# alvinliu0/HumanGaussian

Measured on AMD Instinct MI355X. Metric: rasterize fwd+bwd Gaussians/sec @1024^2, 100k pts, higher is better.
Workload: dtype f32

## Files before the change

### humangaussian_amd/csrc/api.hip

```cpp
#include "hgs_common.h"
#include <stdio.h>
#include <stdlib.h>
#include <algorithm>
#include <atomic>
#include <mutex>

#ifdef HGS_TIMELINE
__device__ unsigned long long hgs_tl[HGS_TL_KERNELS][HGS_TL_SLOTS][4];
#endif
#include "preprocess.hip"
#include "binning.hip"
#include "render_fwd.hip"
#include "knn.hip"
#include "mesh.hip"
#include "fields.hip"
#include "bookkeeping.hip"
#include "optim.hip"

extern "C" __global__ void hgs_k_render_bwd(View, Layout, const hgs_status*, const SortRec*, const float*,
                                            const float*, const float*, const float*, const float*,
                                            const float*, const float*, float*, uint32_t);
extern "C" __global__ void hgs_k_pair_reduce_em(View, Layout, const hgs_status*, const SortRec*, const float*, float*, uint32_t, uint32_t);
extern "C" __global__ void hgs_k_pair_reduce_ch(View, Layout, const hgs_status*, const SortRec*, const float*, float*, uint32_t, uint32_t);

// ... 92 lines not shown
  const BinCarve b = carve_bin(cap);
  char* gp = static_cast<char*>(geom);
  char* bp = static_cast<char*>(bin);
  Layout L;
  L.geom = reinterpret_cast<GeomRec*>(gp + g.geom);
  L.tile_n = reinterpret_cast<uint32_t*>(gp + g.tile_n);
  L.tile_start = reinterpret_cast<uint32_t*>(gp + g.tile_start);
  L.tile_order = reinterpret_cast<uint32_t*>(gp + g.tile_order);
  L.tile_rec = reinterpret_cast<uint4*>(gp + g.tile_rec);
  L.cell_info = reinterpret_cast<CellInfo*>(gp + g.cell_info);
  L.items_part = reinterpret_cast<uint4*>(gp + g.items_part);
  L.fwd_cells = reinterpret_cast<uint32_t*>(gp + g.fwd_cells);
  L.hist = reinterpret_cast<uint32_t*>(gp + g.hist);
  L.tile_gbase = reinterpret_cast<uint32_t*>(gp + g.tile_gbase);
  L.tile_count = reinterpret_cast<uint32_t*>(gp + g.tile_count);
  L.chunk_sums = reinterpret_cast<uint32_t*>(gp + g.chunk_sums);
  L.chunk_base = reinterpret_cast<uint32_t*>(gp + g.chunk_base);
  L.ctr = reinterpret_cast<Counters*>(gp + g.ctr);
  L.keys = bp ? reinterpret_cast<unsigned long long*>(bp + b.keys) : nullptr;
  L.recs = bp ? reinterpret_cast<SortRec*>(bp + b.recs) : nullptr;
  L.cell_list = bp ? reinterpret_cast<uint2*>(bp + b.cell_list) : nullptr;
  L.entpair = bp ? reinterpret_cast<uint2*>(bp + b.entpair) : nullptr;
  L.cstate = bp ? reinterpret_cast<float*>(bp + b.cstate) : nullptr;
  L.items_full = bp ? reinterpret_cast<uint4*>(bp + b.items_full) : nullptr;
  L.full_cap = (uint32_t)((size_t)(cap > 0 ? cap : 0) * HGS_PAIRS_PER_ENTRY / HGS_SEGLEN + 1);
  L.n_contrib = static_cast<uint32_t*>(img);
  return L;
}

View make_view(const hgs_settings* s, int B, int P, int M, int64_t cap, int max_tile_hint = 0, int act = 0) {
// ... 47 lines not shown
#define HGS_STAGE(k)                                                              \
  do {                                                                            \
    if (stage_events && stage_events[k]) {                                        \
      hipError_t e__ = hipEventRecord(static_cast<hipEvent_t>(stage_events[k]), stream); \
      if (e__ != hipSuccess) return hip_rc(e__);                                  \
    }                                                                             \
  } while (0)

struct SideStream {
  std::mutex mu;
  hipStream_t s = nullptr;
  hipEvent_t fork = nullptr, join = nullptr;
  bool tried = false, ok = false;
};

struct DeviceState {
  std::atomic<int> cus;
  SideStream side;
  std::atomic<int> lds_raised[HGS_PRE_BWD_ROWS];
};
DeviceState g_devices[64];
DeviceState* device_state(hipStream_t stream) {
  int dev = 0;
  if (hipStreamGetDevice(stream, &dev) != hipSuccess || dev < 0 || dev >= 64) { (void)hipGetLastError(); return nullptr; }
  return &g_devices[dev];
}
struct DeviceCurrent {
  int dev, cur = 0;
  bool ok, switched;
  explicit DeviceCurrent(const DeviceState* ds)
      : dev((int)(ds - g_devices)), ok(hipGetDevice(&cur) == hipSuccess), switched(ok && cur != dev) {
    if (switched) ok = hipSetDevice(dev) == hipSuccess;
  }
  ~DeviceCurrent() { if (switched) (void)hipSetDevice(cur); }
};

int cu_count(DeviceState* ds) {
  if (!ds) return 256;
  int cus = ds->cus.load(std::memory_order_relaxed);
  if (cus > 0) return cus;
  if (hipDeviceGetAttribute(&cus, hipDeviceAttributeMultiprocessorCount, (int)(ds - g_devices)) != hipSuccess || cus < 1) cus = 256;
  ds->cus.store(cus, std::memory_order_relaxed);
  return cus;
}

SideStream* side_stream(DeviceState* ds) {
  if (!ds) return nullptr;
  SideStream& t = ds->side;
  std::lock_guard<std::mutex> lk(t.mu);
  if (!t.tried) {
    t.tried = true;
    DeviceCurrent on(ds);
    t.ok = on.ok && hipStreamCreateWithFlags(&t.s, hipStreamNonBlocking) == hipSuccess &&
           hipEventCreateWithFlags(&t.fork, hipEventDisableTiming) == hipSuccess &&
           hipEventCreateWithFlags(&t.join, hipEventDisableTiming) == hipSuccess;
    if (!t.ok) (void)hipGetLastError();
  }
  return t.ok ? &t : nullptr;
// ... 215 lines not shown
    if ((shs != nullptr) == (colors_precomp != nullptr)) return HGS_ESHAPE;
    const bool has_sr = scales != nullptr && rotations != nullptr;
    if ((scales != nullptr) != (rotations != nullptr)) return HGS_ESHAPE;
    if (has_sr == (cov3D_precomp != nullptr)) return HGS_ESHAPE;
    if (shs && M < (s->sh_degree + 1) * (s->sh_degree + 1)) return HGS_ESHAPE;
    if (entry_capacity > 0 && !bin) return HGS_EINVAL;
    if ((int64_t)B * P >= (1ll << 31) || P >= (1 << 28)) return HGS_EINVAL;
  }
  if (entry_capacity > HGS_MAX_ENTRY_CAPACITY) return HGS_EINVAL;
  hipStream_t stream = static_cast<hipStream_t>(stream_);
  DeviceState* const ds = device_state(stream);
  const int ncu = cu_count(ds);
  const bool aa = (activation_flags & HGS_ANTIALIAS) != 0;
  const View v = make_view(s, B, P, M, entry_capacity, max_tile_entries_hint > 0 ? max_tile_entries_hint : 0,
                           activation_flags & 7);
  const Layout L = make_layout(geom, bin, img, B, P, v.H, v.W, entry_capacity);
  hgs_status* status_dev =
      reinterpret_cast<hgs_status*>(static_cast<char*>(geom) + carve_geom(B, P, v.H, v.W).status);

  HGS_STAGE(0);
  hipError_t e = hipSuccess;
  if (v.nblk == 0) {
    e = hipMemsetAsync(L.ctr, 0, sizeof(Counters), stream);
    if (e != hipSuccess) return hip_rc(e);
  }
  const size_t lds_bytes = (size_t)v.T * 4;
  if (!v.lds_bins) {
    e = hipMemsetAsync(L.tile_count, 0, (size_t)v.TT * 4, stream);
    if (e != hipSuccess) return hip_rc(e);
  }
  if (v.nblk > 0) {
    if (v.lds_bins)
      hipLaunchKernelGGL(aa ? hgs_k_preprocess_fwd_aa : hgs_k_preprocess_fwd, dim3(v.B * v.nwg), dim3(HGS_BLOCK), lds_bytes,
                         stream, v, L, means3D, shs, colors_precomp, opacities, scales, rotations,
                         cov3D_precomp, radii, means2D_leaf);
    else
      hipLaunchKernelGGL(aa ? hgs_k_preprocess_fwd_ga_aa : hgs_k_preprocess_fwd_ga, dim3(v.B * v.nblk), dim3(HGS_BLOCK), 0,
                         stream, v, L, means3D, shs, colors_precomp, opacities, scales, rotations,
                         cov3D_precomp, radii, means2D_leaf);
    HGS_LAUNCH_CHECK();
  }
  HGS_STAGE(1);
  const unsigned bpv = (unsigned)((v.T + HGS_TILES_PER_WG - 1) / HGS_TILES_PER_WG);
  hipLaunchKernelGGL(hgs_k_tiles, dim3(bpv * (unsigned)v.B), dim3(64 * HGS_ROW_GROUPS), 0, stream, v, L);
  HGS_LAUNCH_CHECK();
  HGS_STAGE(2);
  const unsigned order_wgs = (unsigned)((v.TT + HGS_BLOCK - 1) / HGS_BLOCK);
  hgs_status* status_mapped = status_host_mapped ? status_host : nullptr;
  const unsigned nbin = entry_capacity > 0 ? (unsigned)(v.B * (v.lds_bins ? v.nwg : v.nblk)) : 0u;
  if (v.lds_bins && nbin)
    hipLaunchKernelGGL(hgs_k_fill, dim3(nbin + order_wgs), dim3(HGS_BLOCK), lds_bytes, stream, v, L, status_dev,
                       status_mapped, (int)nbin);
  else
    hipLaunchKernelGGL(hgs_k_fill_ga, dim3(nbin + order_wgs), dim3(HGS_BLOCK), 0, stream, v, L, status_dev,
                       status_mapped, (int)nbin);
  HGS_LAUNCH_CHECK();
  if (status_host && !status_host_mapped) {
    e = hipMemcpyAsync(status_host, status_dev, sizeof(hgs_status), hipMemcpyDeviceToHost, stream);
    if (e != hipSuccess) return hip_rc(e);
  }
// ... 44 lines not shown
    }
  } else {
    HGS_STAGE(3);
  }
  HGS_STAGE(4);
  {
    const int64_t cells = std::min<int64_t>((int64_t)16 * v.TT, (int64_t)HGS_PAIRS_PER_ENTRY * entry_capacity);
    const int64_t fwd_blocks = (int64_t)hgs_knob("HGS_FWD_BLOCKS_PER_CU", 4) * ncu;
    const unsigned cell_blocks = (unsigned)std::max<int64_t>(4, std::min<int64_t>(fwd_blocks, (cells + 3) / 4) & ~int64_t(3));
    const unsigned bg_blocks = (unsigned)v.TT;
    hipLaunchKernelGGL(store_bwd_state ? hgs_k_render_fwd_store : hgs_k_render_fwd_nostore, dim3(cell_blocks + bg_blocks),
                       dim3(HGS_FWD_THREADS), 0, stream, v, L, cell_blocks, status_dev, status_mapped, L.recs, L.cstate,
                       out_color, out_depth, out_alpha);
  }
  HGS_LAUNCH_CHECK();
  HGS_STAGE(5);
  return HGS_OK;
}

int hgs_forward_batch(const hgs_settings* s, int32_t B, int32_t P, int32_t M, const float* means3D,
                      const float* shs, const float* colors_precomp, const float* opacities,
                      const float* scales, const float* rotations, const float* cov3D_precomp,
                      float* out_color, float* out_depth, float* out_alpha, int32_t* radii,
                      void* geom, void* bin, int64_t entry_capacity, void* img,
                      int32_t store_bwd_state, int32_t max_tile_entries_hint, hgs_status* status_host,
                      int32_t status_host_mapped, void* status_event, void* const* stage_events,
                      void* stream_) {
  return hgs_forward_batch_act(s, B, P, M, means3D, shs, colors_precomp, opacities, scales, rotations, cov3D_precomp,
                               out_color, out_depth, out_alpha, radii, geom, bin, entry_capacity, img, store_bwd_state,
                               max_tile_entries_hint, status_host, status_host_mapped, status_event, stage_events, 0,
// ... 546 lines not shown
```

### humangaussian_amd/csrc/binning.hip

```cpp
#include "hgs_common.h"

extern "C" __global__ void __launch_bounds__(64 * HGS_ROW_GROUPS)
hgs_k_tiles(View v, Layout L) {
  __shared__ uint32_t gt[HGS_ROW_GROUPS][HGS_TILES_PER_WG];
  __shared__ uint32_t start_s[HGS_TILES_PER_WG];
  __shared__ uint32_t cls_s[HGS_NCLS];
  const int tid = threadIdx.x, tl = tid & 63;
  const int rg = __builtin_amdgcn_readfirstlane(tid >> 6);
  const int bpv = (v.T + HGS_TILES_PER_WG - 1) / HGS_TILES_PER_WG;
  const int b = (int)blockIdx.x / bpv;
  const int t = ((int)blockIdx.x % bpv) * HGS_TILES_PER_WG + tl;
  const bool valid = t < v.T;
  const size_t g = (size_t)b * v.T + t;
  if (tid < HGS_NCLS) cls_s[tid] = 0;
  uint32_t run = 0;
  if (v.lds_bins) {
    const int rpg = (v.nwg + HGS_ROW_GROUPS - 1) / HGS_ROW_GROUPS;
    const int r0 = rg * rpg, r1 = min(v.nwg, r0 + rpg);
    if (valid) {
      uint32_t* col = L.hist + (size_t)b * v.nwg * v.T + t;
      constexpr int BR = 16;
      for (int r = r0; r < r1; r += BR) {
        uint32_t c[BR];
#pragma unroll
        for (int k = 0; k < BR; ++k) c[k] = (r + k < r1) ? col[(size_t)(r + k) * v.T] : 0u;
#pragma unroll
        for (int k = 0; k < BR; ++k) {
          if (r + k < r1 && c[k]) col[(size_t)(r + k) * v.T] = run;
          run += c[k];
        }
      }
    }
  } else if (rg == 0 && valid) {
    run = L.tile_count[g];
    L.tile_count[g] = 0;
  }
  gt[rg][tl] = run;
  __syncthreads();
  uint32_t gbase = 0;
#pragma unroll
  for (int k = 0; k < HGS_ROW_GROUPS; ++k) gbase += (k < rg) ? gt[k][tl] : 0u;
  if (rg == 0) {
    uint32_t n = 0;
#pragma unroll
    for (int k = 0; k < HGS_ROW_GROUPS; ++k) n += gt[k][tl];
    if (!valid) n = 0;
    const uint32_t i0 = hgs_wave_incl_scan(n);
    unsigned long long b_eb = 0;
    if (tl == 63 && i0) b_eb = atomicAdd(&L.ctr->alloc_eb, (unsigned long long)i0);
    const uint32_t s0 = (uint32_t)__builtin_amdgcn_readlane((int)(uint32_t)b_eb, 63);
    const uint32_t start = s0 + i0 - n;
    start_s[tl] = start;
    if (valid) {
      L.tile_n[g] = n;
      L.tile_start[g] = start;
    }
    const unsigned long long eb = __ballot(valid && n == 0);
    if (tl == 0 && eb) atomicAdd(&cls_s[0], (uint32_t)__popcll(eb));
    if (valid && n) atomicAdd(&cls_s[32 - __clz(n)], 1u);
    const uint32_t mx = hgs_wave_max_u32(n);
    if (tl == 0 && mx) atomicMax(&L.ctr->max_n, mx);
  }
  __syncthreads();
  if (v.lds_bins && valid) L.tile_gbase[(size_t)rg * v.TT + g] = start_s[tl] + gbase;
  if (tid < HGS_NCLS && cls_s[tid]) atomicAdd(&L.ctr->cls_hist[tid].v, cls_s[tid]);

}

__device__ __forceinline__ uint32_t overflow_from_counters(const View& v, const Layout& L) {
  const uint32_t R = (uint32_t)L.ctr->alloc_eb;
  uint32_t o = (R > v.entry_capacity) ? 1u : 0u;
  if (v.max_tile_hint > 0 && L.ctr->max_n > (uint32_t)v.max_tile_hint) o |= 2u;
  return o;
}

__device__ __forceinline__ void place_tiles(const View& v, const Layout& L, int blk, int nblks,
                                            hgs_status* __restrict__ status,
                                            hgs_status* __restrict__ status_host) {
  __shared__ uint32_t cls_base[HGS_NCLS];
  __shared__ uint32_t cls_cnt[HGS_NCLS];
  const int tid = threadIdx.x, lane = tid & 63;
  if (tid < HGS_NCLS) cls_cnt[tid] = L.ctr->cls_hist[tid].v;
  __syncthreads();
  if (tid == 0) {
    uint32_t acc = 0;
    for (int c = HGS_NCLS - 1; c >= 0; --c) { cls_base[c] = acc; acc += cls_cnt[c]; }
  }
  if (blk == 0 && tid == 64) {
    const unsigned long long a_eb = L.ctr->alloc_eb;
    hgs_status st;
    st.num_rendered = (uint32_t)a_eb;
    st.active_tiles = (uint32_t)v.TT - cls_cnt[0];
    st.num_pairs = 0;
    st.bwd_groups = 0;
    st.overflow = overflow_from_counters(v, L);
    st.reserved[0] = v.entry_capacity;
    st.reserved[1] = L.ctr->max_n;
    st.reserved[2] = 1;
    *status = st;
    if (status_host) {
      volatile uint32_t* hs = reinterpret_cast<volatile uint32_t*>(status_host);
      const uint32_t* sw = reinterpret_cast<const uint32_t*>(&st);
      for (int k = 0; k < 7; ++k) hs[k] = sw[k];
      __threadfence_system();
      hs[7] = 1u;
      __threadfence_system();
    }
  }
  if (tid >= 128 && tid < 192) {
    const int nchunk = v.B * v.nblk;
    const int per_wg = (nchunk + nblks - 1) / nblks;
    const int c_begin = blk * per_wg, c_end = min(nchunk, c_begin + per_wg);
    for (int c0 = c_begin; c0 < c_end; c0 += 64) {
      const int c = c0 + lane;
      const uint32_t sum = (c < c_end) ? L.chunk_sums[c] : 0u;
      const uint32_t inc = hgs_wave_incl_scan(sum);
      uint32_t base = 0;
      if (lane == 63 && inc) base = atomicAdd(&L.ctr->entry_alloc, inc);
      base = (uint32_t)__builtin_amdgcn_readlane((int)base, 63);
      if (c < c_end) L.chunk_base[c] = base + inc - sum;
    }
  }
  __syncthreads();
  const int g = blk * HGS_BLOCK + tid;
  const bool valid = g < v.TT;
  const uint32_t n = valid ? L.tile_n[g] : 0u;
  const int c = (valid && n) ? 32 - __clz(n) : 0;
  int leader_of = 0;
  uint32_t rank = 0, cnt = 0;
  unsigned long long todo = __ballot(valid);
  while (todo) {
    const int leader = (int)__builtin_ctzll(todo);
    const int cl = __builtin_amdgcn_readlane(c, leader);
    const unsigned long long same = __ballot(valid && c == cl);
    if (valid && c == cl) {
      leader_of = leader;
      rank = __builtin_amdgcn_mbcnt_hi((uint32_t)(same >> 32), __builtin_amdgcn_mbcnt_lo((uint32_t)same, 0u));
      cnt = (uint32_t)__popcll(same);
    }
    todo &= ~same;
  }
  uint32_t base = 0;
  if (valid && lane == leader_of) base = atomicAdd(&L.ctr->cls_cur[c].v, cnt);
  base = (uint32_t)__shfl((int)base, leader_of, 64);
  const uint32_t pos = cls_base[c] + base + rank;
  if (!valid) return;
  L.tile_order[pos] = (uint32_t)g;
  L.tile_rec[pos] = make_uint4((uint32_t)g, n, L.tile_start[g], 0u);
}

extern "C" __global__ void __launch_bounds__(HGS_BLOCK)
hgs_k_fill(View v, Layout L, hgs_status* __restrict__ status, hgs_status* __restrict__ status_host, int nbin) {
  extern __shared__ __attribute__((aligned(16))) uint32_t lds_cur[];
  if ((int)blockIdx.x >= nbin) {
    place_tiles(v, L, (int)blockIdx.x - nbin, (int)gridDim.x - nbin, status, status_host);
    return;
  }
  if (overflow_from_counters(v, L)) return;
  const int b = (int)blockIdx.x / v.nwg, lw = (int)blockIdx.x % v.nwg;
  const uint32_t* __restrict__ base_row = L.hist + (size_t)blockIdx.x * v.T;
  const int rpg = (v.nwg + HGS_ROW_GROUPS - 1) / HGS_ROW_GROUPS;
  const uint32_t* __restrict__ grp_row = L.tile_gbase + (size_t)(lw / rpg) * v.TT + (size_t)b * v.T;
  for (int t = threadIdx.x; t < v.T; t += HGS_BLOCK) lds_cur[t] = grp_row[t] + base_row[t];
  __syncthreads();
  const GeomRec* __restrict__ geom = L.geom + (size_t)b * v.P;
  for (int c = 0; c < v.cpw; ++c) {
    const int chunk = lw * v.cpw + c;
    if (chunk >= v.nblk) break;
    const int i = chunk * HGS_BLOCK + threadIdx.x;
    if (i >= v.P) continue;
    const uint4 q2 = reinterpret_cast<const uint4*>(&geom[i])[2];
    const uint32_t depth_bits = q2.y, lo = q2.z, hi = q2.w;
    const int minx = lo & 0xffffu, miny = lo >> 16, maxx = hi & 0xffffu, maxy = hi >> 16;
    const unsigned long long key_hi = (unsigned long long)depth_bits << 32;
    for (int ty = miny; ty < maxy; ++ty)
      for (int tx = minx; tx < maxx; ++tx) {
        const uint32_t slot = atomicAdd(&lds_cur[ty * v.grid_x + tx], 1u);
        L.keys[slot] = key_hi | (uint32_t)i;
      }
  }
}

extern "C" __global__ void __launch_bounds__(HGS_BLOCK)
hgs_k_fill_ga(View v, Layout L, hgs_status* __restrict__ status, hgs_status* __restrict__ status_host, int nbin) {
  if ((int)blockIdx.x >= nbin) {
    place_tiles(v, L, (int)blockIdx.x - nbin, (int)gridDim.x - nbin, status, status_host);
// ... 406 lines not shown
#define HGS_RANK_BUCKET_MAX 192
#define HGS_RANK_NB_MAX 2048
#define HGS_SORT_NT 256
#define HGS_SORT_WAVES_PER_EU 3
#define HGS_RANK_GU 2

namespace {

#ifdef HGS_TIMELINE
__shared__ unsigned long long hgs_s_tq[8];
#define HGS_TQ(i) { if (threadIdx.x == 0) hgs_s_tq[(i)] = wall_clock64(); }
#else
#define HGS_TQ(i) {}
#endif

__device__ __forceinline__ void lds_barrier() { asm volatile("s_waitcnt lgkmcnt(0)\n\ts_barrier" ::: "memory"); }

struct __attribute__((aligned(16))) RankLds {
  uint32_t hist[HGS_RANK_NB_MAX + 1];
  uint32_t wtot[16];
  uint32_t tot16[8];
  uint32_t dmin, dmax, maxcnt, pad;
};
static_assert(sizeof(uint32_t) * (HGS_RANK_NB_MAX + 1) >= sizeof(uint16_t) * 4096, "the masks of the longest list fit into the histogram");

template <int NT>
__device__ __forceinline__ void bucket_scan(RankLds& R, uint32_t NB) {
  int tid = (int)threadIdx.x;
  asm volatile("" : "+v"(tid));
  const int lane = tid & 63, wv = tid >> 6;
  const uint32_t PER = NB / (uint32_t)NT;
// ... 546 lines not shown
```

### humangaussian_amd/csrc/hgs_common.h

```cpp
#pragma once
#include <hip/hip_runtime.h>
#include <stdint.h>

#include "../../include/hgs_rast.h"
#include "cellmask.h"
#include "entryrec.h"

#define HGS_TILE 16
#define HGS_TILE_PIX 256
#define HGS_BLOCK 256
#define HGS_ROW_GROUPS 16
#define HGS_TILES_PER_WG 64
#define HGS_RB 16
#define HGS_ROW_F4 (HGS_RB * HGS_REC_F4 + 1)
#define HGS_BWD_BLOCK_WAVES 12
#define HGS_SEGLEN 128
#define HGS_NEAR_Z 0.2f
#define HGS_ALPHA_MIN (1.0f / 255.0f)
#define HGS_ALPHA_MAX 0.99f
#define HGS_T_EPS 0.0001f
#define HGS_CSTATE_FLOATS (6 * 16)
#define HGS_ROW_FLOATS 12
#define HGS_GROW_F4 (HGS_ROW_FLOATS / 4)
#define HGS_PROW_FLOATS 10
// ... 44 lines not shown

__host__ __device__ __forceinline__ uint32_t hgs_cell_class(uint32_t len) {
  const uint32_t nb = (len + HGS_RB - 1) / HGS_RB;
  return nb >= 33u ? 0u : nb >= 25u ? 1u : nb >= 17u ? 2u : nb >= 13u ? 3u : nb >= 9u ? 4u : nb >= 7u ? 5u : nb >= 5u ? 6u : 11u - nb;
}

struct Layout {
  GeomRec* geom;
  uint32_t* tile_n;
  uint32_t* tile_start;
  uint32_t* tile_order;
  uint4* tile_rec;
  uint32_t* hist;
  uint32_t* tile_gbase;
  uint32_t* tile_count;
  uint32_t* chunk_sums;
  uint32_t* chunk_base;
  CellInfo* cell_info;
  uint32_t* fwd_cells;
  uint4* items_part;
  Counters* ctr;
  unsigned long long* keys;
  SortRec* recs;
  uint2* cell_list;
  uint2* entpair;
  float* cstate;
  uint32_t full_cap;
  uint4* items_full;
  uint32_t* n_contrib;
};
// ... 53 lines not shown
  x += __builtin_amdgcn_update_dpp(0, x, HGS_DPP_ROW_SHR(4), 0xf, 0xf, false);
  x += __builtin_amdgcn_update_dpp(0, x, HGS_DPP_ROW_SHR(8), 0xf, 0xf, false);
  x += __builtin_amdgcn_update_dpp(0, x, HGS_DPP_ROW_BCAST15, 0xa, 0xf, false);
  x += __builtin_amdgcn_update_dpp(0, x, HGS_DPP_ROW_BCAST31, 0xc, 0xf, false);
  return (uint32_t)x;
}

__device__ __forceinline__ uint32_t hgs_wave_max_u32(uint32_t v) {
  int x = (int)v;
  x = (int)max((uint32_t)x, (uint32_t)__builtin_amdgcn_update_dpp(0, x, HGS_DPP_ROW_SHR(1), 0xf, 0xf, false));
  x = (int)max((uint32_t)x, (uint32_t)__builtin_amdgcn_update_dpp(0, x, HGS_DPP_ROW_SHR(2), 0xf, 0xf, false));
  x = (int)max((uint32_t)x, (uint32_t)__builtin_amdgcn_update_dpp(0, x, HGS_DPP_ROW_SHR(4), 0xf, 0xf, false));
  x = (int)max((uint32_t)x, (uint32_t)__builtin_amdgcn_update_dpp(0, x, HGS_DPP_ROW_SHR(8), 0xf, 0xf, false));
  x = (int)max((uint32_t)x, (uint32_t)__builtin_amdgcn_update_dpp(0, x, HGS_DPP_ROW_BCAST15, 0xa, 0xf, false));
  x = (int)max((uint32_t)x, (uint32_t)__builtin_amdgcn_update_dpp(0, x, HGS_DPP_ROW_BCAST31, 0xc, 0xf, false));
  return (uint32_t)__builtin_amdgcn_readlane(x, 63);
}

template <int NT>
__device__ __forceinline__ uint32_t hgs_block_excl_scan(uint32_t v, uint32_t* wtot,
                                                        uint32_t& total) {
  const int lane = threadIdx.x & 63, w = threadIdx.x >> 6;
  const uint32_t incl = hgs_wave_incl_scan(v);
  __syncthreads();
  if (lane == 63) wtot[w] = incl;
  __syncthreads();
  uint32_t base = 0, tot = 0;
#pragma unroll
  for (int k = 0; k < NT / 64; ++k) {
    const uint32_t t = wtot[k];
// ... 44 lines not shown
```

### humangaussian_amd/csrc/preprocess.hip

```cpp
#include "hgs_common.h"

namespace {

__device__ __constant__ const float SH_C0 = 0.28209479177387814f;
__device__ __constant__ const float SH_C1 = 0.4886025119029199f;
__device__ __constant__ const float SH_C2[5] = {1.0925484305920792f, -1.0925484305920792f,
                                                0.31539156525252005f, -1.0925484305920792f,
                                                0.5462742152960396f};
__device__ __constant__ const float SH_C3[7] = {-0.5900435899266435f, 2.890611442640554f,
                                                -0.4570457994644658f, 0.3731763325901154f,
                                                -0.4570457994644658f, 1.445305721320277f,
                                                -0.5900435899266435f};

struct Cov3 { float c0, c1, c2, c3, c4, c5; };

struct RotScale {
  float R00, R01, R02, R10, R11, R12, R20, R21, R22;
  float sx, sy, sz;
};

__device__ __forceinline__ float act_opacity(float raw, int act) {
  return (act & HGS_ACT_OPACITY_SIGMOID) ? 1.0f / (1.0f + expf(-raw)) : raw;
}
__device__ __forceinline__ void act_scale(const float* __restrict__ scales, int i, int act, float& s0, float& s1, float& s2) {
// ... 279 lines not shown
    }
    rec.r = col[0]; rec.g = col[1]; rec.b = col[2];
    rec.clamped = cl;
  }
  return (uint32_t)tight_area;
}

__device__ __forceinline__ void store_geom(GeomRec* dstp, const GeomRec& rec) {
  uint4* dst = reinterpret_cast<uint4*>(dstp);
  const uint4* src = reinterpret_cast<const uint4*>(&rec);
  dst[0] = src[0]; dst[1] = src[1]; dst[2] = src[2]; dst[3] = src[3];
}

}

__device__ __forceinline__ uint32_t chunk_prefix(uint32_t tt, uint32_t* wtot, uint32_t* chunk_sum) {
  uint32_t total;
  const uint32_t ex = hgs_block_excl_scan<HGS_BLOCK>(tt, wtot, total);
  if (threadIdx.x == 0) *chunk_sum = total;
  return ex;
}

__device__ __forceinline__ void zero_counters(const Layout& L) {
  if (blockIdx.x == 0)
    for (uint32_t i = threadIdx.x; i < sizeof(Counters) / 4; i += blockDim.x) reinterpret_cast<uint32_t*>(L.ctr)[i] = 0u;
}

template <bool AA>
__device__ __forceinline__ void preprocess_fwd_body(
    const View& v, const Layout& L, const float* __restrict__ means3D, const float* __restrict__ shs,
    const float* __restrict__ colors_precomp, const float* __restrict__ opacities, const float* __restrict__ scales,
    const float* __restrict__ rotations, const float* __restrict__ cov3D_precomp, int32_t* __restrict__ radii,
    float* __restrict__ zero_leaf) {
  extern __shared__ __attribute__((aligned(16))) uint32_t lds_hist[];
  __shared__ uint32_t wtot[HGS_BLOCK / 64];
  zero_counters(L);
  const int b = (int)blockIdx.x / v.nwg, lw = (int)blockIdx.x % v.nwg;
  const Cam cam = v.cam[b];
  for (int t = threadIdx.x; t < v.T; t += HGS_BLOCK) lds_hist[t] = 0u;
  __syncthreads();
  const int gxm = v.grid_x;
  for (int c = 0; c < v.cpw; ++c) {
    const int chunk = lw * v.cpw + c;
    if (chunk >= v.nblk) break;
    const int i = chunk * HGS_BLOCK + threadIdx.x;
    uint32_t tt = 0;
    if (i < v.P) {
      GeomRec rec;
      tt = preprocess_one<AA>(v, cam, i, means3D, shs, colors_precomp, opacities, scales, rotations,
                              cov3D_precomp, rec);
      radii[(size_t)b * v.P + i] = rec.radius;
      if (zero_leaf) {
        float* z = zero_leaf + ((size_t)b * v.P + i) * 3;
        z[0] = 0.0f; z[1] = 0.0f; z[2] = 0.0f;
      }
      store_geom(&L.geom[(size_t)b * v.P + i], rec);
      if (tt) {
        const int minx = rec.rect_lo & 0xffffu, miny = rec.rect_lo >> 16;
        const int maxx = rec.rect_hi & 0xffffu, maxy = rec.rect_hi >> 16;
        for (int ty = miny; ty < maxy; ++ty)
          for (int tx = minx; tx < maxx; ++tx) atomicAdd(&lds_hist[ty * gxm + tx], 1u);
      }
    }
    const uint32_t off = chunk_prefix(tt, wtot, &L.chunk_sums[(size_t)b * v.nblk + chunk]);
    if (i < v.P && tt) L.geom[(size_t)b * v.P + i].offset = off;
  }
  __syncthreads();
  uint32_t* row = L.hist + (size_t)blockIdx.x * v.T;
  for (int t = threadIdx.x; t < v.T; t += HGS_BLOCK) row[t] = lds_hist[t];
}

template <bool AA>
__device__ __forceinline__ void preprocess_fwd_ga_body(
    const View& v, const Layout& L, const float* __restrict__ means3D, const float* __restrict__ shs,
    const float* __restrict__ colors_precomp, const float* __restrict__ opacities, const float* __restrict__ scales,
    const float* __restrict__ rotations, const float* __restrict__ cov3D_precomp, int32_t* __restrict__ radii,
    float* __restrict__ zero_leaf) {
  __shared__ uint32_t wtot[HGS_BLOCK / 64];
  zero_counters(L);
  const int b = (int)blockIdx.x / v.nblk, chunk = (int)blockIdx.x % v.nblk;
  const Cam cam = v.cam[b];
  const int i = chunk * HGS_BLOCK + threadIdx.x;
  uint32_t tt = 0;
  if (i < v.P) {
// ... 2 lines not shown
                            cov3D_precomp, rec);
    radii[(size_t)b * v.P + i] = rec.radius;
    if (zero_leaf) {
      float* z = zero_leaf + ((size_t)b * v.P + i) * 3;
      z[0] = 0.0f; z[1] = 0.0f; z[2] = 0.0f;
    }
    store_geom(&L.geom[(size_t)b * v.P + i], rec);
    if (tt) {
      const int minx = rec.rect_lo & 0xffffu, miny = rec.rect_lo >> 16;
      const int maxx = rec.rect_hi & 0xffffu, maxy = rec.rect_hi >> 16;
      uint32_t* cnt = L.tile_count + (size_t)b * v.T;
      for (int ty = miny; ty < maxy; ++ty)
        for (int tx = minx; tx < maxx; ++tx) atomicAdd(&cnt[ty * v.grid_x + tx], 1u);
    }
  }
  const uint32_t off = chunk_prefix(tt, wtot, &L.chunk_sums[blockIdx.x]);
  if (i < v.P && tt) L.geom[(size_t)b * v.P + i].offset = off;
}

#define HGS_PRE_FWD_KERNEL(NAME, BODY, AA)                                                                       \
  extern "C" __global__ void __launch_bounds__(HGS_BLOCK) NAME(                                                  \
      View v, Layout L, const float* __restrict__ means3D, const float* __restrict__ shs,                        \
      const float* __restrict__ colors_precomp, const float* __restrict__ opacities,                             \
      const float* __restrict__ scales, const float* __restrict__ rotations,                                     \
      const float* __restrict__ cov3D_precomp, int32_t* __restrict__ radii, float* __restrict__ zero_leaf) {     \
    BODY<AA>(v, L, means3D, shs, colors_precomp, opacities, scales, rotations, cov3D_precomp, radii, zero_leaf);   \
  }
HGS_PRE_FWD_KERNEL(hgs_k_preprocess_fwd, preprocess_fwd_body, false)
HGS_PRE_FWD_KERNEL(hgs_k_preprocess_fwd_ga, preprocess_fwd_ga_body, false)
HGS_PRE_FWD_KERNEL(hgs_k_preprocess_fwd_aa, preprocess_fwd_body, true)
HGS_PRE_FWD_KERNEL(hgs_k_preprocess_fwd_ga_aa, preprocess_fwd_ga_body, true)
// ... 543 lines not shown
```

### humangaussian_amd/csrc/render_fwd.hip

```cpp
#include "hgs_common.h"

namespace {

typedef float hgs_fwd_f32x2 __attribute__((ext_vector_type(2)));

struct PixState {
  hgs_fwd_f32x2 C01, C2D;
  float Wt;
  float T;
  uint32_t last;
};

__device__ __forceinline__ void blend_one(PixState& s, float pxf, float pyf, const float4 r0,
                                          const float4 r1, const float4 r2) {
  float G, alpha, m2, m3;
  const bool keep = hgs_eval_alpha(r0.x - pxf, r0.y - pyf, r0.z, r0.w, r1.x, r1.y, G, alpha, m2, m3);
  const float ak = keep ? alpha : 0.0f;
  const float test_T = s.T * (1.0f - ak);
  const bool ok = test_T >= HGS_T_EPS;
  const float wgt = ok ? ak * s.T : 0.0f;
  s.T = ok ? test_T : -__builtin_fabsf(s.T);
  const bool upd = keep && ok;
  const hgs_fwd_f32x2 rg = {r1.z, r1.w}, bd = {r2.x, r2.y}, w2 = {wgt, wgt};
  s.C01 = __builtin_elementwise_fma(rg, w2, s.C01);
// ... 290 lines not shown
  out_depth[o1 + pix] = 0.0f;
  out_alpha[o1 + pix] = 0.0f;
  L.n_contrib[o1 + pix] = 0u;
}

#define HGS_RENDER_FWD_KERNEL(NAME, STORE)                                                                 \
  extern "C" __global__ void __launch_bounds__(HGS_FWD_THREADS) NAME(                                       \
      View v, Layout L, uint32_t cell_blocks, hgs_status* __restrict__ status,                               \
      hgs_status* __restrict__ status_host, const SortRec* __restrict__ recs, float* __restrict__ cstate, float* __restrict__ out_color,           \
      float* __restrict__ out_depth, float* __restrict__ out_alpha) {                                        \
    __shared__ float4 s_rec[HGS_FWD_THREADS / 64][4 * HGS_ROW_F4];        \
    __shared__ __attribute__((aligned(16))) uint32_t s_pre[HGS_NFC * HGS_FWD_PRE_STRIDE];                    \
    const bool overflow = status->overflow != 0;                                                             \
    if (blockIdx.x >= cell_blocks) {                                                                         \
      const uint32_t g = blockIdx.x - cell_blocks;                                                           \
      if (g < (uint32_t)v.TT) render_fwd_background(v, L, overflow, (int)g, out_color, out_depth, out_alpha); \
      return;                                                                                                \
    }                                                                                                        \
    if (overflow) return;                                                                                    \
    if (blockIdx.x == 0 && threadIdx.x == 0) {        \
      const uint32_t np = (uint32_t)L.ctr->alloc_ps;                                                         \
      status->num_pairs = np;                                                                                \
      if (status_host) *reinterpret_cast<volatile uint32_t*>(&status_host->num_pairs) = np;                  \
    }                                                                                                        \
    HGS_TL_BEGIN();                                                                                          \
    const int w = __builtin_amdgcn_readfirstlane((int)threadIdx.x >> 6);                                     \
     \
    const size_t dcap = hgs_die_cells(v.TT);                                                                 \
    if (threadIdx.x < HGS_NFC) {                                                                             \
      uint32_t acc = 0;                                                                                      \
// ... 36 lines not shown
```

Before: 655.3 million.

## Replace tile-count kernel with atomic per-tile claims in preprocess for LDS bins

In the LDS-bins path, each preprocess workgroup now claims its per-tile base offsets with atomicAdd into a persistent per-stream counter buffer and adds its entry total to a per-view total. This lets the separate hgs_k_tiles launch be dropped. The fill kernel builds tile starts with an in-block prefix scan, place_tiles derives tile_n, tile_start, class histograms and the overflow check itself, and the forward render's background blocks zero the counters for the next call. The aim is to remove a kernel launch and a column-scan pass over the histogram. In exchange it adds global atomics, redundant full-tile scans in every fill and place block, host-side mutex and map bookkeeping, and per-stream device allocations.

Result: slower. 639.0 million (-2.5%).

```diff
diff --git a/humangaussian_amd/csrc/api.hip b/humangaussian_amd/csrc/api.hip
--- a/humangaussian_amd/csrc/api.hip
+++ b/humangaussian_amd/csrc/api.hip
@@ -3,6 +3,8 @@
 #include <stdlib.h>
 #include <algorithm>
 #include <atomic>
+#include <map>
+#include <memory>
 #include <mutex>
 
 #ifdef HGS_TIMELINE
@@ -130,6 +132,7 @@
   L.hist = reinterpret_cast<uint32_t*>(gp + g.hist);
   L.tile_gbase = reinterpret_cast<uint32_t*>(gp + g.tile_gbase);
   L.tile_count = reinterpret_cast<uint32_t*>(gp + g.tile_count);
+  L.view_tot = nullptr;
   L.chunk_sums = reinterpret_cast<uint32_t*>(gp + g.chunk_sums);
   L.chunk_base = reinterpret_cast<uint32_t*>(gp + g.chunk_base);
   L.ctr = reinterpret_cast<Counters*>(gp + g.ctr);
@@ -207,10 +210,19 @@
   bool tried = false, ok = false;
 };
 
+struct ClaimCounters {
+  std::mutex mu;
+  uint32_t* p = nullptr;
+  size_t words = 0;
+  bool dirty = false;
+};
+
 struct DeviceState {
   std::atomic<int> cus;
   SideStream side;
   std::atomic<int> lds_raised[HGS_PRE_BWD_ROWS];
+  std::mutex claims_mu;
+  std::map<hipStream_t, std::unique_ptr<ClaimCounters>> claims;
 };
 DeviceState g_devices[64];
 DeviceState* device_state(hipStream_t stream) {
@@ -235,6 +247,35 @@
   if (hipDeviceGetAttribute(&cus, hipDeviceAttributeMultiprocessorCount, (int)(ds - g_devices)) != hipSuccess || cus < 1) cus = 256;
   ds->cus.store(cus, std::memory_order_relaxed);
   return cus;
+}
+
+ClaimCounters* claim_counters(DeviceState* ds, hipStream_t stream) {
+  if (!ds) return nullptr;
+  std::lock_guard<std::mutex> lk(ds->claims_mu);
+  std::unique_ptr<ClaimCounters>& c = ds->claims[stream];
+  if (!c) c.reset(new ClaimCounters());
+  return c.get();
+}
+hipError_t claim_counters_ready(DeviceState* ds, ClaimCounters* c, size_t words, hipStream_t stream) {
+  if (c->words < words) {
+    DeviceCurrent on(ds);
+    if (!on.ok) return hipErrorInvalidDevice;
+    size_t want = (size_t)HGS_MAX_VIEWS + 16384;
+    while (want < words) want *= 2;
+    uint32_t* p = nullptr;
+    hipError_t e = hipMalloc(reinterpret_cast<void**>(&p), want * 4);
+    if (e != hipSuccess) return e;
+    if (c->p) (void)hipFree(c->p);
+    c->p = p;
+    c->words = want;
+    c->dirty = true;
+  }
+  if (c->dirty) {
+    const hipError_t e = hipMemsetAsync(c->p, 0, c->words * 4, stream);
+    if (e != hipSuccess) return e;
+    c->dirty = false;
+  }
+  return hipSuccess;
 }
 
 SideStream* side_stream(DeviceState* ds) {
@@ -480,12 +521,23 @@
   const bool aa = (activation_flags & HGS_ANTIALIAS) != 0;
   const View v = make_view(s, B, P, M, entry_capacity, max_tile_entries_hint > 0 ? max_tile_entries_hint : 0,
                            activation_flags & 7);
-  const Layout L = make_layout(geom, bin, img, B, P, v.H, v.W, entry_capacity);
+  Layout L = make_layout(geom, bin, img, B, P, v.H, v.W, entry_capacity);
   hgs_status* status_dev =
       reinterpret_cast<hgs_status*>(static_cast<char*>(geom) + carve_geom(B, P, v.H, v.W).status);
 
+  hipError_t e = hipSuccess;
+  ClaimCounters* const claim = v.lds_bins ? claim_counters(ds, stream) : nullptr;
+  std::unique_lock<std::mutex> claim_lk;
+  if (v.lds_bins) {
+    if (!claim) return hip_rc(hipErrorInvalidDevice);
+    claim_lk = std::unique_lock<std::mutex>(claim->mu);
+    e = claim_counters_ready(ds, claim, (size_t)HGS_MAX_VIEWS + (size_t)v.TT, stream);
+    if (e != hipSuccess) return hip_rc(e);
+    L.view_tot = claim->p;
+    L.tile_count = claim->p + HGS_MAX_VIEWS;
+    claim->dirty = true;
+  }
   HGS_STAGE(0);
-  hipError_t e = hipSuccess;
   if (v.nblk == 0) {
     e = hipMemsetAsync(L.ctr, 0, sizeof(Counters), stream);
     if (e != hipSuccess) return hip_rc(e);
@@ -507,9 +559,11 @@
     HGS_LAUNCH_CHECK();
   }
   HGS_STAGE(1);
-  const unsigned bpv = (unsigned)((v.T + HGS_TILES_PER_WG - 1) / HGS_TILES_PER_WG);
-  hipLaunchKernelGGL(hgs_k_tiles, dim3(bpv * (unsigned)v.B), dim3(64 * HGS_ROW_GROUPS), 0, stream, v, L);
-  HGS_LAUNCH_CHECK();
+  if (!v.lds_bins) {
+    const unsigned bpv = (unsigned)((v.T + HGS_TILES_PER_WG - 1) / HGS_TILES_PER_WG);
+    hipLaunchKernelGGL(hgs_k_tiles, dim3(bpv * (unsigned)v.B), dim3(64 * HGS_ROW_GROUPS), 0, stream, v, L);
+    HGS_LAUNCH_CHECK();
+  }
   HGS_STAGE(2);
   const unsigned order_wgs = (unsigned)((v.TT + HGS_BLOCK - 1) / HGS_BLOCK);
   hgs_status* status_mapped = status_host_mapped ? status_host : nullptr;
@@ -584,6 +638,7 @@
                        out_color, out_depth, out_alpha);
   }
   HGS_LAUNCH_CHECK();
+  if (claim) claim->dirty = false;
   HGS_STAGE(5);
   return HGS_OK;
 }
diff --git a/humangaussian_amd/csrc/binning.hip b/humangaussian_amd/csrc/binning.hip
--- a/humangaussian_amd/csrc/binning.hip
+++ b/humangaussian_amd/csrc/binning.hip
@@ -1,9 +1,9 @@
 #include "hgs_common.h"
+
+__device__ __forceinline__ void lds_barrier() { asm volatile("s_waitcnt lgkmcnt(0)\n\ts_barrier" ::: "memory"); }
 
 extern "C" __global__ void __launch_bounds__(64 * HGS_ROW_GROUPS)
 hgs_k_tiles(View v, Layout L) {
-  __shared__ uint32_t gt[HGS_ROW_GROUPS][HGS_TILES_PER_WG];
-  __shared__ uint32_t start_s[HGS_TILES_PER_WG];
   __shared__ uint32_t cls_s[HGS_NCLS];
   const int tid = threadIdx.x, tl = tid & 63;
   const int rg = __builtin_amdgcn_readfirstlane(tid >> 6);
@@ -13,44 +13,18 @@
   const bool valid = t < v.T;
   const size_t g = (size_t)b * v.T + t;
   if (tid < HGS_NCLS) cls_s[tid] = 0;
-  uint32_t run = 0;
-  if (v.lds_bins) {
-    const int rpg = (v.nwg + HGS_ROW_GROUPS - 1) / HGS_ROW_GROUPS;
-    const int r0 = rg * rpg, r1 = min(v.nwg, r0 + rpg);
-    if (valid) {
-      uint32_t* col = L.hist + (size_t)b * v.nwg * v.T + t;
-      constexpr int BR = 16;
-      for (int r = r0; r < r1; r += BR) {
-        uint32_t c[BR];
-#pragma unroll
-        for (int k = 0; k < BR; ++k) c[k] = (r + k < r1) ? col[(size_t)(r + k) * v.T] : 0u;
-#pragma unroll
-        for (int k = 0; k < BR; ++k) {
-          if (r + k < r1 && c[k]) col[(size_t)(r + k) * v.T] = run;
-          run += c[k];
-        }
-      }
-    }
-  } else if (rg == 0 && valid) {
-    run = L.tile_count[g];
-    L.tile_count[g] = 0;
-  }
-  gt[rg][tl] = run;
   __syncthreads();
-  uint32_t gbase = 0;
-#pragma unroll
-  for (int k = 0; k < HGS_ROW_GROUPS; ++k) gbase += (k < rg) ? gt[k][tl] : 0u;
   if (rg == 0) {
     uint32_t n = 0;
-#pragma unroll
-    for (int k = 0; k < HGS_ROW_GROUPS; ++k) n += gt[k][tl];
-    if (!valid) n = 0;
+    if (valid) {
+      n = L.tile_count[g];
+      L.tile_count[g] = 0;
+    }
     const uint32_t i0 = hgs_wave_incl_scan(n);
     unsigned long long b_eb = 0;
     if (tl == 63 && i0) b_eb = atomicAdd(&L.ctr->alloc_eb, (unsigned long long)i0);
     const uint32_t s0 = (uint32_t)__builtin_amdgcn_readlane((int)(uint32_t)b_eb, 63);
     const uint32_t start = s0 + i0 - n;
-    start_s[tl] = start;
     if (valid) {
       L.tile_n[g] = n;
       L.tile_start[g] = start;
@@ -62,16 +36,27 @@
     if (tl == 0 && mx) atomicMax(&L.ctr->max_n, mx);
   }
   __syncthreads();
-  if (v.lds_bins && valid) L.tile_gbase[(size_t)rg * v.TT + g] = start_s[tl] + gbase;
   if (tid < HGS_NCLS && cls_s[tid]) atomicAdd(&L.ctr->cls_hist[tid].v, cls_s[tid]);
-
-}
-
+}
+
+
+__device__ __forceinline__ uint32_t overflow_word(const View& v, uint32_t R, uint32_t max_n) {
+  uint32_t o = (R > v.entry_capacity) ? 1u : 0u;
+  if (v.max_tile_hint > 0 && max_n > (uint32_t)v.max_tile_hint) o |= 2u;
+  return o;
+}
 __device__ __forceinline__ uint32_t overflow_from_counters(const View& v, const Layout& L) {
-  const uint32_t R = (uint32_t)L.ctr->alloc_eb;
-  uint32_t o = (R > v.entry_capacity) ? 1u : 0u;
-  if (v.max_tile_hint > 0 && L.ctr->max_n > (uint32_t)v.max_tile_hint) o |= 2u;
-  return o;
+  return overflow_word(v, (uint32_t)L.ctr->alloc_eb, L.ctr->max_n);
+}
+__device__ __forceinline__ uint32_t entries_of_call(const View& v, const Layout& L, int b, uint32_t& before_view) {
+  unsigned long long R = 0;
+  before_view = 0;
+  for (int k = 0; k < v.B; ++k) {
+    const uint32_t x = L.view_tot[k];
+    if (k < b) before_view += x;
+    R += x;
+  }
+  return R > 0xffffffffull ? 0xffffffffu : (uint32_t)R;
 }
 
 __device__ __forceinline__ void place_tiles(const View& v, const Layout& L, int blk, int nblks,
@@ -79,23 +64,118 @@
                                             hgs_status* __restrict__ status_host) {
   __shared__ uint32_t cls_base[HGS_NCLS];
   __shared__ uint32_t cls_cnt[HGS_NCLS];
-  const int tid = threadIdx.x, lane = tid & 63;
-  if (tid < HGS_NCLS) cls_cnt[tid] = L.ctr->cls_hist[tid].v;
-  __syncthreads();
+  __shared__ uint32_t red_s[3][HGS_BLOCK / 64];
+  const int tid = threadIdx.x, lane = tid & 63, wv = __builtin_amdgcn_readfirstlane(tid >> 6);
+  const int g = blk * HGS_BLOCK + tid;
+  const bool valid = g < v.TT;
+  const int nchunk = v.B * v.nblk;
+  const int per_wg = (nchunk + nblks - 1) / nblks;
+  const int c_begin = blk * per_wg, c_end = min(nchunk, c_begin + per_wg);
+  uint32_t ch_sum = 0, ch_inc = 0, ch_base = 0;
+  if (wv == 2 && c_begin + lane < c_end) ch_sum = L.chunk_sums[c_begin + lane];
+  uint32_t n = 0, start = 0;
+  if (v.lds_bins) {
+    if (valid) n = L.tile_count[g];
+  } else if (valid) {
+    n = L.tile_n[g];
+    start = L.tile_start[g];
+  }
+  if (tid < HGS_NCLS) cls_cnt[tid] = v.lds_bins ? 0u : L.ctr->cls_hist[tid].v;
+  if (wv == 2) {
+    ch_inc = hgs_wave_incl_scan(ch_sum);
+    if (lane == 63 && ch_inc) ch_base = atomicAdd(&L.ctr->entry_alloc, ch_inc);
+  }
+  const int c = (valid && n) ? 32 - __clz(n) : 0;
+  int leader_of = 0;
+  uint32_t rank = 0, cnt = 0;
+  {
+    unsigned long long todo = __ballot(valid);
+    while (todo) {
+      const int leader = (int)__builtin_ctzll(todo);
+      const int cl = __builtin_amdgcn_readlane(c, leader);
+      const unsigned long long same = __ballot(valid && c == cl);
+      if (valid && c == cl) {
+        leader_of = leader;
+        rank = __builtin_amdgcn_mbcnt_hi((uint32_t)(same >> 32), __builtin_amdgcn_mbcnt_lo((uint32_t)same, 0u));
+        cnt = (uint32_t)__popcll(same);
+      }
+      todo &= ~same;
+    }
+  }
+  uint32_t base = 0;
+  if (valid && lane == leader_of) base = atomicAdd(&L.ctr->cls_cur[c].v, cnt);
+  lds_barrier();
+  uint32_t R, max_n;
+  if (v.lds_bins) {
+    uint32_t before = 0, mx = 0;
+    constexpr int TB = 16;
+    const int nit = (v.TT + HGS_BLOCK - 1) / HGS_BLOCK;
+    for (int it0 = 0; it0 < nit; it0 += TB) {
+      uint32_t nn[TB];
+#pragma unroll
+      for (int k = 0; k < TB; ++k) {
+        const int gg = (it0 + k) * HGS_BLOCK + tid;
+        nn[k] = gg < v.TT ? L.tile_count[gg] : 0u;
+      }
+      int cc[TB];
+      uint32_t present = 0, present32 = 0;
+#pragma unroll
+      for (int k = 0; k < TB; ++k) {
+        const bool in = (it0 + k) * HGS_BLOCK + tid < v.TT;
+        if (it0 + k < blk) before += nn[k];
+        mx = max(mx, nn[k]);
+        cc[k] = in ? (nn[k] ? 32 - __clz(nn[k]) : 0) : -1;
+        if (in) { if (cc[k] < 32) present |= 1u << cc[k]; else present32 = 1u; }
+      }
+      present = hgs_wave_or_u32(present);
+      present32 = hgs_wave_or_u32(present32);
+      for (int cl = 0; cl <= 32; ++cl) {
+        if (!(cl < 32 ? (present >> cl) & 1u : present32)) continue;
+        uint32_t cnt = 0;
+#pragma unroll
+        for (int k = 0; k < TB; ++k) cnt += (uint32_t)__popcll(__ballot(cc[k] == cl));
+        if (lane == 0) atomicAdd(&cls_cnt[cl], cnt);
+      }
+    }
+    const uint32_t inc = hgs_wave_incl_scan(n);
+    const uint32_t wbefore = (uint32_t)__builtin_amdgcn_readlane((int)hgs_wave_incl_scan(before), 63);
+    mx = hgs_wave_max_u32(mx);
+    if (lane == 63) { red_s[0][wv] = wbefore; red_s[1][wv] = mx; red_s[2][wv] = inc; }
+    lds_barrier();
+    start = inc - n;
+    max_n = 0;
+#pragma unroll
+    for (int k = 0; k < HGS_BLOCK / 64; ++k) {
+      start += red_s[0][k] + (k < wv ? red_s[2][k] : 0u);
+      max_n = max(max_n, red_s[1][k]);
+    }
+    uint32_t unused;
+    R = entries_of_call(v, L, 0, unused);
+    if (valid) {
+      L.tile_n[g] = n;
+      L.tile_start[g] = start;
+    }
+  } else {
+    R = (uint32_t)L.ctr->alloc_eb;
+    max_n = L.ctr->max_n;
+  }
   if (tid == 0) {
     uint32_t acc = 0;
-    for (int c = HGS_NCLS - 1; c >= 0; --c) { cls_base[c] = acc; acc += cls_cnt[c]; }
+    for (int k = HGS_NCLS - 1; k >= 0; --k) { cls_base[k] = acc; acc += cls_cnt[k]; }
   }
   if (blk == 0 && tid == 64) {
-    const unsigned long long a_eb = L.ctr->alloc_eb;
+    if (v.lds_bins) {
+      L.ctr->alloc_eb = R;
+      L.ctr->max_n = max_n;
+    }
     hgs_status st;
-    st.num_rendered = (uint32_t)a_eb;
+    st.num_rendered = R;
     st.active_tiles = (uint32_t)v.TT - cls_cnt[0];
     st.num_pairs = 0;
     st.bwd_groups = 0;
-    st.overflow = overflow_from_counters(v, L);
+    st.overflow = overflow_word(v, R, max_n);
     st.reserved[0] = v.entry_capacity;
-    st.reserved[1] = L.ctr->max_n;
+    st.reserved[1] = max_n;
     st.reserved[2] = 1;
     *status = st;
     if (status_host) {
@@ -107,69 +187,91 @@
       __threadfence_system();
     }
   }
-  if (tid >= 128 && tid < 192) {
-    const int nchunk = v.B * v.nblk;
-    const int per_wg = (nchunk + nblks - 1) / nblks;
-    const int c_begin = blk * per_wg, c_end = min(nchunk, c_begin + per_wg);
-    for (int c0 = c_begin; c0 < c_end; c0 += 64) {
-      const int c = c0 + lane;
-      const uint32_t sum = (c < c_end) ? L.chunk_sums[c] : 0u;
+  if (wv == 2) {
+    ch_base = (uint32_t)__builtin_amdgcn_readlane((int)ch_base, 63);
+    if (c_begin + lane < c_end) L.chunk_base[c_begin + lane] = ch_base + ch_inc - ch_sum;
+    for (int c0 = c_begin + 64; c0 < c_end; c0 += 64) {
+      const int ch = c0 + lane;
+      const uint32_t sum = (ch < c_end) ? L.chunk_sums[ch] : 0u;
       const uint32_t inc = hgs_wave_incl_scan(sum);
-      uint32_t base = 0;
-      if (lane == 63 && inc) base = atomicAdd(&L.ctr->entry_alloc, inc);
-      base = (uint32_t)__builtin_amdgcn_readlane((int)base, 63);
-      if (c < c_end) L.chunk_base[c] = base + inc - sum;
-    }
-  }
-  __syncthreads();
-  const int g = blk * HGS_BLOCK + tid;
-  const bool valid = g < v.TT;
-  const uint32_t n = valid ? L.tile_n[g] : 0u;
-  const int c = (valid && n) ? 32 - __clz(n) : 0;
-  int leader_of = 0;
-  uint32_t rank = 0, cnt = 0;
-  unsigned long long todo = __ballot(valid);
-  while (todo) {
-    const int leader = (int)__builtin_ctzll(todo);
-    const int cl = __builtin_amdgcn_readlane(c, leader);
-    const unsigned long long same = __ballot(valid && c == cl);
-    if (valid && c == cl) {
-      leader_of = leader;
-      rank = __builtin_amdgcn_mbcnt_hi((uint32_t)(same >> 32), __builtin_amdgcn_mbcnt_lo((uint32_t)same, 0u));
-      cnt = (uint32_t)__popcll(same);
-    }
-    todo &= ~same;
-  }
-  uint32_t base = 0;
-  if (valid && lane == leader_of) base = atomicAdd(&L.ctr->cls_cur[c].v, cnt);
+      uint32_t b0 = 0;
+      if (lane == 63 && inc) b0 = atomicAdd(&L.ctr->entry_alloc, inc);
+      b0 = (uint32_t)__builtin_amdgcn_readlane((int)b0, 63);
+      if (ch < c_end) L.chunk_base[ch] = b0 + inc - sum;
+    }
+  }
+  lds_barrier();
   base = (uint32_t)__shfl((int)base, leader_of, 64);
   const uint32_t pos = cls_base[c] + base + rank;
   if (!valid) return;
   L.tile_order[pos] = (uint32_t)g;
-  L.tile_rec[pos] = make_uint4((uint32_t)g, n, L.tile_start[g], 0u);
-}
+  L.tile_rec[pos] = make_uint4((uint32_t)g, n, start, 0u);
+}
+
+#define HGS_FILL_SWEEP 16
+static_assert(HGS_FILL_SWEEP * (HGS_BLOCK / 64) == 64, "one wave scans the (round, wave) totals of a sweep");
 
 extern "C" __global__ void __launch_bounds__(HGS_BLOCK)
 hgs_k_fill(View v, Layout L, hgs_status* __restrict__ status, hgs_status* __restrict__ status_host, int nbin) {
   extern __shared__ __attribute__((aligned(16))) uint32_t lds_cur[];
+  __shared__ uint32_t part_s[2][64];
+  __shared__ uint32_t max_s[HGS_BLOCK / 64];
   if ((int)blockIdx.x >= nbin) {
     place_tiles(v, L, (int)blockIdx.x - nbin, (int)gridDim.x - nbin, status, status_host);
     return;
   }
-  if (overflow_from_counters(v, L)) return;
+  const int tid = (int)threadIdx.x, lane = tid & 63, wv = __builtin_amdgcn_readfirstlane(tid >> 6);
   const int b = (int)blockIdx.x / v.nwg, lw = (int)blockIdx.x % v.nwg;
+  const GeomRec* __restrict__ geom = L.geom + (size_t)b * v.P;
+  auto chunk_q2 = [&](int c) {
+    const int chunk = lw * v.cpw + c, i = chunk * HGS_BLOCK + tid;
+    return (c < v.cpw && chunk < v.nblk && i < v.P) ? reinterpret_cast<const uint4*>(&geom[i])[2] : make_uint4(0u, 0u, 0u, 0u);
+  };
+  uint4 q2n = chunk_q2(0);
   const uint32_t* __restrict__ base_row = L.hist + (size_t)blockIdx.x * v.T;
-  const int rpg = (v.nwg + HGS_ROW_GROUPS - 1) / HGS_ROW_GROUPS;
-  const uint32_t* __restrict__ grp_row = L.tile_gbase + (size_t)(lw / rpg) * v.TT + (size_t)b * v.T;
-  for (int t = threadIdx.x; t < v.T; t += HGS_BLOCK) lds_cur[t] = grp_row[t] + base_row[t];
-  __syncthreads();
-  const GeomRec* __restrict__ geom = L.geom + (size_t)b * v.P;
+  const uint32_t* __restrict__ tot = L.tile_count + (size_t)b * v.T;
+  uint32_t carry;
+  const uint32_t R = entries_of_call(v, L, b, carry);
+  uint32_t vmax = 0;
+  for (int s0 = 0, buf = 0; s0 < v.T; s0 += HGS_FILL_SWEEP * HGS_BLOCK, buf ^= 1) {
+    uint32_t n[HGS_FILL_SWEEP], br[HGS_FILL_SWEEP], inc[HGS_FILL_SWEEP];
+#pragma unroll
+    for (int k = 0; k < HGS_FILL_SWEEP; ++k) {
+      const int t = s0 + k * HGS_BLOCK + tid;
+      n[k] = t < v.T ? tot[t] : 0u;
+      br[k] = t < v.T ? base_row[t] : 0u;
+    }
+#pragma unroll
+    for (int k = 0; k < HGS_FILL_SWEEP; ++k) {
+      inc[k] = hgs_wave_incl_scan(n[k]);
+      vmax = max(vmax, n[k]);
+      if (lane == 63) part_s[buf][k * (HGS_BLOCK / 64) + wv] = inc[k];
+    }
+    lds_barrier();
+    const uint32_t x = part_s[buf][lane];
+    const uint32_t xi = hgs_wave_incl_scan(x), xe = xi - x;
+#pragma unroll
+    for (int k = 0; k < HGS_FILL_SWEEP; ++k) {
+      const int t = s0 + k * HGS_BLOCK + tid;
+      const uint32_t before = (uint32_t)__shfl((int)xe, k * (HGS_BLOCK / 64) + wv, 64);
+      if (t < v.T) lds_cur[t] = carry + before + inc[k] - n[k] + br[k];
+    }
+    carry += (uint32_t)__builtin_amdgcn_readlane((int)xi, 63);
+  }
+  vmax = hgs_wave_max_u32(vmax);
+  if (lane == 0) max_s[wv] = vmax;
+  lds_barrier();
+  uint32_t view_max = 0;
+#pragma unroll
+  for (int k = 0; k < HGS_BLOCK / 64; ++k) view_max = max(view_max, max_s[k]);
+  if (overflow_word(v, R, view_max)) return;
   for (int c = 0; c < v.cpw; ++c) {
     const int chunk = lw * v.cpw + c;
     if (chunk >= v.nblk) break;
-    const int i = chunk * HGS_BLOCK + threadIdx.x;
+    const int i = chunk * HGS_BLOCK + tid;
+    const uint4 q2 = q2n;
+    q2n = chunk_q2(c + 1);
     if (i >= v.P) continue;
-    const uint4 q2 = reinterpret_cast<const uint4*>(&geom[i])[2];
     const uint32_t depth_bits = q2.y, lo = q2.z, hi = q2.w;
     const int minx = lo & 0xffffu, miny = lo >> 16, maxx = hi & 0xffffu, maxy = hi >> 16;
     const unsigned long long key_hi = (unsigned long long)depth_bits << 32;
@@ -606,7 +708,6 @@
 #define HGS_TQ(i) {}
 #endif
 
-__device__ __forceinline__ void lds_barrier() { asm volatile("s_waitcnt lgkmcnt(0)\n\ts_barrier" ::: "memory"); }
 
 struct __attribute__((aligned(16))) RankLds {
   uint32_t hist[HGS_RANK_NB_MAX + 1];
diff --git a/humangaussian_amd/csrc/hgs_common.h b/humangaussian_amd/csrc/hgs_common.h
--- a/humangaussian_amd/csrc/hgs_common.h
+++ b/humangaussian_amd/csrc/hgs_common.h
@@ -82,6 +82,7 @@
   uint32_t* hist;
   uint32_t* tile_gbase;
   uint32_t* tile_count;
+  uint32_t* view_tot;
   uint32_t* chunk_sums;
   uint32_t* chunk_base;
   CellInfo* cell_info;
@@ -165,6 +166,17 @@
   x = (int)max((uint32_t)x, (uint32_t)__builtin_amdgcn_update_dpp(0, x, HGS_DPP_ROW_SHR(8), 0xf, 0xf, false));
   x = (int)max((uint32_t)x, (uint32_t)__builtin_amdgcn_update_dpp(0, x, HGS_DPP_ROW_BCAST15, 0xa, 0xf, false));
   x = (int)max((uint32_t)x, (uint32_t)__builtin_amdgcn_update_dpp(0, x, HGS_DPP_ROW_BCAST31, 0xc, 0xf, false));
+  return (uint32_t)__builtin_amdgcn_readlane(x, 63);
+}
+
+__device__ __forceinline__ uint32_t hgs_wave_or_u32(uint32_t v) {
+  int x = (int)v;
+  x |= __builtin_amdgcn_update_dpp(0, x, HGS_DPP_ROW_SHR(1), 0xf, 0xf, false);
+  x |= __builtin_amdgcn_update_dpp(0, x, HGS_DPP_ROW_SHR(2), 0xf, 0xf, false);
+  x |= __builtin_amdgcn_update_dpp(0, x, HGS_DPP_ROW_SHR(4), 0xf, 0xf, false);
+  x |= __builtin_amdgcn_update_dpp(0, x, HGS_DPP_ROW_SHR(8), 0xf, 0xf, false);
+  x |= __builtin_amdgcn_update_dpp(0, x, HGS_DPP_ROW_BCAST15, 0xa, 0xf, false);
+  x |= __builtin_amdgcn_update_dpp(0, x, HGS_DPP_ROW_BCAST31, 0xc, 0xf, false);
   return (uint32_t)__builtin_amdgcn_readlane(x, 63);
 }
 
diff --git a/humangaussian_amd/csrc/preprocess.hip b/humangaussian_amd/csrc/preprocess.hip
--- a/humangaussian_amd/csrc/preprocess.hip
+++ b/humangaussian_amd/csrc/preprocess.hip
@@ -317,8 +317,7 @@
 
 }
 
-__device__ __forceinline__ uint32_t chunk_prefix(uint32_t tt, uint32_t* wtot, uint32_t* chunk_sum) {
-  uint32_t total;
+__device__ __forceinline__ uint32_t chunk_prefix(uint32_t tt, uint32_t* wtot, uint32_t* chunk_sum, uint32_t& total) {
   const uint32_t ex = hgs_block_excl_scan<HGS_BLOCK>(tt, wtot, total);
   if (threadIdx.x == 0) *chunk_sum = total;
   return ex;
@@ -343,6 +342,7 @@
   for (int t = threadIdx.x; t < v.T; t += HGS_BLOCK) lds_hist[t] = 0u;
   __syncthreads();
   const int gxm = v.grid_x;
+  uint32_t wg_total = 0;
   for (int c = 0; c < v.cpw; ++c) {
     const int chunk = lw * v.cpw + c;
     if (chunk >= v.nblk) break;
@@ -365,12 +365,29 @@
           for (int tx = minx; tx < maxx; ++tx) atomicAdd(&lds_hist[ty * gxm + tx], 1u);
       }
     }
-    const uint32_t off = chunk_prefix(tt, wtot, &L.chunk_sums[(size_t)b * v.nblk + chunk]);
+    uint32_t total;
+    const uint32_t off = chunk_prefix(tt, wtot, &L.chunk_sums[(size_t)b * v.nblk + chunk], total);
+    wg_total += total;
     if (i < v.P && tt) L.geom[(size_t)b * v.P + i].offset = off;
   }
   __syncthreads();
+  if (threadIdx.x == 0 && wg_total) atomicAdd(&L.view_tot[b], wg_total);
   uint32_t* row = L.hist + (size_t)blockIdx.x * v.T;
-  for (int t = threadIdx.x; t < v.T; t += HGS_BLOCK) row[t] = lds_hist[t];
+  uint32_t* claim = L.tile_count + (size_t)b * v.T;
+  constexpr int CLAIMS = 16;
+  for (int t0 = threadIdx.x; t0 < v.T; t0 += CLAIMS * HGS_BLOCK) {
+    uint32_t n[CLAIMS], base[CLAIMS];
+#pragma unroll
+    for (int k = 0; k < CLAIMS; ++k) {
+      const int t = t0 + k * HGS_BLOCK;
+      n[k] = t < v.T ? lds_hist[t] : 0u;
+    }
+#pragma unroll
+    for (int k = 0; k < CLAIMS; ++k) base[k] = n[k] ? atomicAdd(&claim[t0 + k * HGS_BLOCK], n[k]) : 0u;
+#pragma unroll
+    for (int k = 0; k < CLAIMS; ++k)
+      if (t0 + k * HGS_BLOCK < v.T) row[t0 + k * HGS_BLOCK] = base[k];
+  }
 }
 
 template <bool AA>
@@ -403,7 +420,8 @@
         for (int tx = minx; tx < maxx; ++tx) atomicAdd(&cnt[ty * v.grid_x + tx], 1u);
     }
   }
-  const uint32_t off = chunk_prefix(tt, wtot, &L.chunk_sums[blockIdx.x]);
+  uint32_t total;
+  const uint32_t off = chunk_prefix(tt, wtot, &L.chunk_sums[blockIdx.x], total);
   if (i < v.P && tt) L.geom[(size_t)b * v.P + i].offset = off;
 }
 
diff --git a/humangaussian_amd/csrc/render_fwd.hip b/humangaussian_amd/csrc/render_fwd.hip
--- a/humangaussian_amd/csrc/render_fwd.hip
+++ b/humangaussian_amd/csrc/render_fwd.hip
@@ -328,6 +328,11 @@
     const bool overflow = status->overflow != 0;                                                             \
     if (blockIdx.x >= cell_blocks) {                                                                         \
       const uint32_t g = blockIdx.x - cell_blocks;                                                           \
+                \
+      if (v.lds_bins && threadIdx.x == 0 && g < (uint32_t)v.TT) {                                            \
+        L.tile_count[g] = 0u;                                                                                \
+        if (g < (uint32_t)v.B) L.view_tot[g] = 0u;                                                           \
+      }                                                                                                      \
       if (g < (uint32_t)v.TT) render_fwd_background(v, L, overflow, (int)g, out_color, out_depth, out_alpha); \
       return;                                                                                                \
     }                                                                                                        \
```
